# hukaixuan19970627/yolov5_obb

Measured on AMD Instinct MI355X. Metric: val.py img/s (hot path: non_max_suppression_obb, bs16) + NMS ms/img @100k cand, DOTAv1.5 1024^2, 1/2/4/8 GPU, higher is better.
Workload: dtype f16; 1 GPU; DOTAv1.5 1024^2 bs16 (BASELINE metric; configs[1] thresholds): yolov5 OBB head output (16,64512,201) fp16, 4 distinct tensors rotated (cold: 1.66 GB working set) -> non_max_suppression_obb (conf .25, iou .45, multi_label, max_det 1500), val.py --task speed hot path = dt[2] of val.py; global_batch=16, anchors_per_image=64512, nc=16, detections_per_batch=3734, parallelism=dp1 (images sharded, no data-path collective)

## Files before the change

yolov5_obb_amd/csrc/obb_device.h:

```cpp
#pragma once
#include <stdint.h>

#if defined(__HIPCC__)
#include <hip/hip_runtime.h>
#define OBB_DEV __device__ __forceinline__
#define OBB_HD __host__ __device__ __forceinline__
#else
#include <math.h>
#define OBB_DEV inline
#define OBB_HD inline
#endif

namespace obb {

constexpr int kWave = 64;

constexpr float f32_next_up(float f) {
  uint32_t u = __builtin_bit_cast(uint32_t, f);
  if (f == 0.0f) return __builtin_bit_cast(float, (uint32_t)1);
  u = (f > 0.0f) ? u + 1 : u - 1;
  return __builtin_bit_cast(float, u);
}
constexpr float f32_next_down(float f) { return -f32_next_up(-f); }
constexpr float f32_ceil(double d) {
  float f = (float)d;
  return ((double)f >= d) ? f : f32_next_up(f);
}
constexpr float f32_floor(double d) {
  float f = (float)d;
  return ((double)f <= d) ? f : f32_next_down(f);
}

static_assert((double)f32_ceil(1e-6) >= 1e-6 && (double)f32_next_down(f32_ceil(1e-6)) < 1e-6, "f32_ceil");
static_assert((double)f32_floor(1e-14) <= 1e-14 && (double)f32_next_up(f32_floor(1e-14)) > 1e-14, "f32_floor");

template <typename F> OBB_HD F min_nan(F a, F b) { return (a != a || b != b) ? a + b : (b < a ? b : a); }
template <typename F> OBB_HD bool box_too_small(F w, F h) { return min_nan(w, h) < F(0.001); }

}
```

yolov5_obb_amd/csrc/riou_device.h:

```cpp
#pragma once
#include "obb_device.h"

namespace obb {

struct RBoxFeat {
  float x, y, w, h;
  float sh, cw, ch, sw;
  float r;
  float c, s;
  float area;
};

OBB_HD RBoxFeat rbox_make_feat(float x, float y, float w, float h, float a) {
  RBoxFeat f;
  double th = (double)a;
  float c2 = (float)cos(th) * 0.5f;
  float s2 = (float)sin(th) * 0.5f;
  f.x = x; f.y = y; f.w = w; f.h = h;
  f.sh = s2 * h; f.cw = c2 * w; f.ch = c2 * h; f.sw = s2 * w;
  f.c = c2 * 2.0f; f.s = s2 * 2.0f;
  f.r = sqrtf(w * w + h * h) * 0.5005f;
  f.area = w * h;
  return f;
}
// ... 182 lines not shown
    for (int j = 0; j < 4; j++) {
      float det = e2x[j] * e1y[i] - e1x[i] * e2y[j];
      if (fabsf(det) <= kDetLe) continue;
      float dx = v2x[j] - v1x[i], dy = v2y[j] - v1y[i];
      float t1 = (e2x[j] * dy - dx * e2y[j]) / det;
      float t2 = (e1x[i] * dy - dx * e1y[i]) / det;
      if (t1 >= 0.0f && t1 <= 1.0f && t2 >= 0.0f && t2 <= 1.0f) {
        if constexpr (STORE) {
          px[n * STRIDE] = v1x[i] + e1x[i] * t1;
          py[n * STRIDE] = v1y[i] + e1y[i] * t1;
        }
        n++;
      }
    }
  }
  {
    float abab = e2x[0] * e2x[0] + e2y[0] * e2y[0];
    float adad = e2x[3] * e2x[3] + e2y[3] * e2y[3];
#pragma unroll
    for (int i = 0; i < 4; i++) {
      float apx = v1x[i] - v2x[0], apy = v1y[i] - v2y[0];
      float apab = apx * e2x[0] + apy * e2y[0];
      float apad = -(apx * e2x[3] + apy * e2y[3]);
      if (apab >= 0 && apad >= 0 && apab <= abab && apad <= adad) {
        if constexpr (STORE) { px[n * STRIDE] = v1x[i]; py[n * STRIDE] = v1y[i]; }
        n++;
      }
    }
  }
  {
    float abab = e1x[0] * e1x[0] + e1y[0] * e1y[0];
    float adad = e1x[3] * e1x[3] + e1y[3] * e1y[3];
#pragma unroll
    for (int i = 0; i < 4; i++) {
      float apx = v2x[i] - v1x[0], apy = v2y[i] - v1y[0];
      float apab = apx * e1x[0] + apy * e1y[0];
      float apad = -(apx * e1x[3] + apy * e1y[3]);
      if (apab >= 0 && apad >= 0 && apab <= abab && apad <= adad) {
        if constexpr (STORE) { px[n * STRIDE] = v2x[i]; py[n * STRIDE] = v2y[i]; }
        n++;
      }
    }
  }
  return n;
}

OBB_HD int rbox_npoints(const RBoxFeat& A, const RBoxFeat& B) {
  constexpr float kAreaLt = f32_ceil(1e-14);
  if (A.area < kAreaLt || B.area < kAreaLt) return -1;
  return rbox_points<1, false>(A, B, nullptr, nullptr);
}

template <int STRIDE>
OBB_HD float rbox_iou(const RBoxFeat& A, const RBoxFeat& B, float* px, float* py) {
  constexpr float kAreaLt = f32_ceil(1e-14);
  constexpr float kCpLtNeg = f32_ceil(-1e-6);
  constexpr float kCpLt = f32_ceil(1e-6);
  constexpr float kD2Gt = f32_floor(1e-8);

  if (A.area < kAreaLt || B.area < kAreaLt) return 0.f;
  const int n = rbox_points<STRIDE, true>(A, B, px, py);

  float inter = 0.f;
  if (n > 2) {
    int t = 0;
    float tx = px[0], ty = py[0];
    for (int i = 1; i < n; i++) {
      float x = px[i * STRIDE], y = py[i * STRIDE];
      if (y < ty || (y == ty && x < tx)) { t = i; tx = x; ty = y; }
    }
    for (int i = 0; i < n; i++) { px[i * STRIDE] -= tx; py[i * STRIDE] -= ty; }
    {
      float x0 = px[0], y0 = py[0];
      px[0] = px[t * STRIDE]; py[0] = py[t * STRIDE];
      px[t * STRIDE] = x0; py[t * STRIDE] = y0;
    }
    for (int i = 1; i < n - 1; i++) {
      float qix = px[i * STRIDE], qiy = py[i * STRIDE];
      for (int j = i + 1; j < n; j++) {
        float qjx = px[j * STRIDE], qjy = py[j * STRIDE];
        float cp = qix * qjy - qjx * qiy;
        bool sw = cp < kCpLtNeg;
        if (!sw && fabsf(cp) < kCpLt) sw = (qix * qix + qiy * qiy) > (qjx * qjx + qjy * qjy);
        if (sw) {
          px[j * STRIDE] = qix; py[j * STRIDE] = qiy;
          qix = qjx; qiy = qjy;
        }
      }
      px[i * STRIDE] = qix; py[i * STRIDE] = qiy;
    }
    int k = 1;
    for (; k < n; k++) {
      float x = px[k * STRIDE], y = py[k * STRIDE];
      if (x * x + y * y > kD2Gt) break;
    }
    if (k < n) {
      px[1 * STRIDE] = px[k * STRIDE]; py[1 * STRIDE] = py[k * STRIDE];
      int m = 2;
      for (int i = k + 1; i < n; i++) {
        float qx = px[i * STRIDE], qy = py[i * STRIDE];
        while (m > 1) {
          float bx2 = px[(m - 2) * STRIDE], by2 = py[(m - 2) * STRIDE];
          float q1x = qx - bx2, q1y = qy - by2;
          float q2x = px[(m - 1) * STRIDE] - bx2, q2y = py[(m - 1) * STRIDE] - by2;
          if (q1x * q2y >= q2x * q1y) m--; else break;
        }
        px[m * STRIDE] = qx; py[m * STRIDE] = qy; m++;
      }
      if (m > 2) {
        float q0x = px[0], q0y = py[0];
        float acc = 0.f;
        float pxx = px[1 * STRIDE] - q0x, pyy = py[1 * STRIDE] - q0y;
        for (int i = 1; i < m - 1; i++) {
          float nx = px[(i + 1) * STRIDE] - q0x, ny = py[(i + 1) * STRIDE] - q0y;
          acc += fabsf(pxx * ny - nx * pyy);
          pxx = nx; pyy = ny;
        }
        inter = acc * 0.5f;
      }
    }
  }
  return inter / (A.area + B.area - inter);
}

}
```

yolov5_obb_amd/csrc/nms.hip:

```cpp
#include <hip/hip_runtime.h>
#include <cstring>
#include <stdint.h>
#include <stdlib.h>
#include <stdio.h>
#include <string.h>
#include <hip/hip_fp16.h>
#include "launch_once.h"
#include "obb_device.h"
#include "nms_core.h"
#include "nms_mk.h"
#include "obb_hip.h"
#include "psrs_sort.h"
#include "nms_small.h"
#include "segsort.h"
#include "ws_layout.h"
#include "nms_plan.h"

namespace obb {

enum { PROF_DECODE = 0, PROF_SEGSORT, PROF_PREP, PROF_STEPS, PROF_GATHER, PROF_NMS_SORT, PROF_NMS_PREP, PROF_NMS_STEPS, PROF_N };
struct ProfState {
  int on = 0;
  static constexpr int kMax = 8192;
  hipEvent_t ev0[kMax], ev1[kMax];
// ... 939 lines not shown
  if (const int rc = head_tta_build(npass, passes_host, dtype, bs, na, no, a_total, &h, nullptr)) return rc;
  return run_nms_obb(nullptr, nullptr, dtype, bs, a_total, no, conf_thres, iou_thres, classes_host, n_classes, agnostic, multi_label, max_det,
                     max_nms, max_wh, extra8, n_extra, cap_img, expected_cand, out, out_packed ? 1 : 0, out_count, status, ws, ws_size,
                     (hipStream_t)stream, state, state_bytes, nullptr, &h);
}

int obb_profile_enable(int on) {
  g_prof.on = on == 2 ? 2 : (on != 0 ? 1 : 0);
  g_prof.used = 0;
  if (g_prof.on) {
    const int want = 2048 < ProfState::kMax ? 2048 : ProfState::kMax;
    while (g_prof.created < want) {
      if (hipEventCreate(&g_prof.ev0[g_prof.created]) != hipSuccess) return OBB_ERR_INTERNAL;
      if (hipEventCreate(&g_prof.ev1[g_prof.created]) != hipSuccess) { hipEventDestroy(g_prof.ev0[g_prof.created]); return OBB_ERR_INTERNAL; }
      g_prof.created++;
    }
  }
  return OBB_OK;
}

int obb_profile_collect(double* ms_sum, int64_t* count, int n_stages) {
  for (int i = 0; i < n_stages; i++) { ms_sum[i] = 0.0; count[i] = 0; }
  for (int k = 0; k < g_prof.used; k++) {
    float ms = 0.f;
    if (hipEventSynchronize(g_prof.ev1[k]) != hipSuccess) return OBB_ERR_INTERNAL;
    if (hipEventElapsedTime(&ms, g_prof.ev0[k], g_prof.ev1[k]) != hipSuccess) return OBB_ERR_INTERNAL;
    const int id = g_prof.id[k];
    if (id < n_stages) { ms_sum[id] += ms; count[id]++; }
  }
  g_prof.used = 0;
  return OBB_OK;
}

int obb_nms_set_max_grid(int max_workgroups) {
  g_max_grid = max_workgroups > 0 ? max_workgroups : 0;
  return OBB_OK;
}

const char* obb_version(void) { return "obb_hip 0.2 (gfx950)"; }

int obb_device_info(int* cu_count, int* wave_size, char* arch_name, int arch_name_len) {
  int dev = 0;
  if (hipGetDevice(&dev) != hipSuccess) return OBB_ERR_NO_DEVICE;
  hipDeviceProp_t p;
  if (hipGetDeviceProperties(&p, dev) != hipSuccess) return OBB_ERR_NO_DEVICE;
  if (cu_count) *cu_count = p.multiProcessorCount;
  if (wave_size) *wave_size = p.warpSize;
  if (arch_name && arch_name_len > 0) { strncpy(arch_name, p.gcnArchName, arch_name_len - 1); arch_name[arch_name_len - 1] = 0; }
  return OBB_OK;
}

}

#ifdef OBB_SMALL_TRACE
extern "C" int obb_debug_small_trace2(unsigned long long* words) {
  static unsigned long long zero2[2048 * 8];
  if (hipDeviceSynchronize() != hipSuccess) return -1;
  if (hipMemcpyFromSymbol(words, HIP_SYMBOL(obb::g_small_trace2), sizeof(obb::g_small_trace2)) != hipSuccess) return -1;
  return hipMemcpyToSymbol(HIP_SYMBOL(obb::g_small_trace2), zero2, sizeof(obb::g_small_trace2)) == hipSuccess ? 0 : -1;
}
extern "C" int obb_debug_small_trace(unsigned long long* seg_words, unsigned long long* tail_words) {
  if (hipDeviceSynchronize() != hipSuccess) return -1;
  if (hipMemcpyFromSymbol(seg_words, HIP_SYMBOL(obb::g_small_trace), sizeof(obb::g_small_trace)) != hipSuccess) return -2;
  if (hipMemcpyFromSymbol(tail_words, HIP_SYMBOL(obb::g_small_trace_tail), sizeof(obb::g_small_trace_tail)) != hipSuccess) return -3;
  static unsigned long long zero[2048 * 16];
  if (hipMemcpyToSymbol(HIP_SYMBOL(obb::g_small_trace), zero, sizeof(obb::g_small_trace)) != hipSuccess) return -4;
  if (hipMemcpyToSymbol(HIP_SYMBOL(obb::g_small_trace_tail), zero, sizeof(obb::g_small_trace_tail)) != hipSuccess) return -5;
  return 0;
}
#endif
```

yolov5_obb_amd/csrc/nms_plan.h:

```cpp
#pragma once
#include <stddef.h>
#include <stdint.h>
#include <stdlib.h>

#include "nms_limits.h"
#include "ws_layout.h"

namespace obb {

enum FbWord {
  kFbSteps = 0,
  kFbKept = 1,
  kFbSlabs = 2,
  kFbEnqueued = 3,
  kFbTicksPersist = 4,
  kFbTicksMk = 5,
  kFbKeptPersist = 6,
  kFbKeptMk = 7,
  kFbWords = 8
};
struct FbSnapshot { int w[kFbWords]; };
static inline FbSnapshot fb_snapshot(const int* words) {
  FbSnapshot s;
  for (int i = 0; i < kFbWords; i++) s.w[i] = *(const volatile int*)(words + i);
// ... 123 lines not shown
    p.slab_cap = sparse ? 2048 : 1024;
  }
  return p;
}

struct SmallHelpBlocks { int *work, *seg_np, *seg_ticket; unsigned long long *part_main, *part_help; };
static inline SmallHelpBlocks small_help_layout(WsCursor& w, int helpers, int64_t nseg, int64_t n_pos) {
  SmallHelpBlocks b;
  b.work = w.take<int>((size_t)helpers);
  b.seg_np = w.take<int>((size_t)nseg); b.seg_ticket = w.take<int>((size_t)nseg);
  b.part_main = w.take<unsigned long long>((size_t)n_pos * kSmallWords);
  b.part_help = w.take<unsigned long long>((size_t)helpers * kSmallMax * kSmallWords);
  return b;
}
static inline size_t small_help_bytes(int helpers, int64_t nseg, int64_t n_pos) {
  WsCursor w(nullptr);
  small_help_layout(w, helpers, nseg, n_pos);
  return w.total();
}

struct ObbPlanIn {
  int64_t bs, A;
  int nc, agnostic, multi_label;
  float iou_thres, max_wh;
  int64_t n_extra;
  int64_t cap_img;
  int64_t max_nms, max_det;
  int64_t expected_cand;
  int out_packed;
  int hw_cus, cus;
  long long ecap;
  size_t sort_tmp_bytes;
  size_t ps_scratch_bytes;
};
struct ObbPlan {
  int ncs;
  int class_ok;
  int multi_label;
  int64_t expected_cand, seg_hint;
  int small_hint;
  int lds_sort;
  int small_nms;
  int self_sort;
  int helpers;
  int fused_out;
  int rows_per_thread;
  int parts;
  int plan_nb, plan_chunk;
  int64_t max_seg;
  unsigned radix_mask;
  int psrs;
  unsigned gparts;
  int window;
};

static inline ObbPlan plan_nms_obb(const ObbPlanIn& in, const NmsEnv& env) {
  ObbPlan p{};
  const int64_t bs = in.bs, cap_img = in.cap_img;
  p.seg_hint = (in.expected_cand >> 32) & 0x1fffffff;
  p.small_hint = ((in.expected_cand >> 62) & 1) != 0;
  p.expected_cand = in.expected_cand & 0xffffffffll;
  p.ncs = in.agnostic ? 1 : in.nc;
  const int64_t nseg = bs * p.ncs;
  p.class_ok = (!in.agnostic && in.nc > 1 && in.A + in.n_extra < (1ll << 24) && in.iou_thres >= 0.f && in.max_wh > 0.f) ? 1 : 0;
  p.multi_label = (in.multi_label && in.nc > 1) ? 1 : 0;
  p.lds_sort = p.expected_cand > 0 && p.expected_cand <= kSortLdsHint;
  p.rows_per_thread = (bs * in.A >= 4LL * kDecThreads * 480) ? 4 : (bs * in.A >= 2LL * kDecThreads * 480) ? 2 : 1;
  p.max_seg = (in.max_nms > 0 && in.max_nms < cap_img) ? in.max_nms : cap_img;
  p.window = nms_window(in.max_det);
  const int nms_capmax = cap_max(nseg);
  p.plan_chunk = kCapFirst < nms_capmax ? kCapFirst : nms_capmax;
  p.small_nms = p.lds_sort && p.class_ok && p.seg_hint > 0 && p.seg_hint <= kSmallMax && in.iou_thres >= 0.f && nseg <= 65535;
  p.plan_nb = (nseg > 1 && !p.small_nms) ? nms_grid(nseg, bs * p.max_seg, kCapFirst, in.cus) : 0;
  const bool self_possible = p.small_nms && !in.out_packed && (int64_t)p.ncs * kSmallMax <= cap_img && env.self_sort != 0;
  if (p.small_nms && !(self_possible && env.self_sort == 2 && env.small_helpers < 0)) {
    const int64_t free_cus = (int64_t)in.hw_cus - nseg;
    p.helpers = env.small_helpers >= 0 ? env.small_helpers : (int)(free_cus < 0 ? 0 : (free_cus > kSmallHelpMax ? kSmallHelpMax : free_cus));
  }
  if (p.helpers > 0) {
    const size_t have = (size_t)(nseg < (int64_t)in.cus ? nseg : (int64_t)in.cus) * (size_t)in.ecap * 4;
    if (small_help_bytes(p.helpers, nseg, bs * cap_img) > have) p.helpers = 0;
  }
  p.self_sort = self_possible && p.helpers == 0;
  if (p.lds_sort) {
    if (!p.self_sort) p.parts = (p.class_ok && p.ncs >= 8) ? 4 : 1;
  } else {
    int tb = 0;
    while ((1ll << tb) < in.A * in.nc + in.n_extra + 1) tb++;
    unsigned mask = 0xF0u;
    for (int d = 0; d < 4; d++) if (tb > d * 8) mask |= 1u << d;
    if (p.class_ok) mask = 0xFFu;
    p.radix_mask = mask;
    p.psrs = bs == 1 && cap_img <= kPsMaxN && in.sort_tmp_bytes >= in.ps_scratch_bytes;
  }
  p.fused_out = p.small_nms && !in.out_packed;
  if (!p.fused_out)
    p.gparts = p.expected_cand <= 2048 ? 1u : (unsigned)((p.expected_cand + 1023) / 1024 > 16 ? 16 : (p.expected_cand + 1023) / 1024);
  return p;
}

}
```

yolov5_obb_amd/csrc/nmsobb_impl.h:

```cpp
#pragma once
#include "dtype_device.h"
#include "obb_device.h"
#include "segsort.h"
#include "nms_plan.h"

namespace obb {

struct ClassMask { unsigned long long w[4]; int all; };

template <typename T> __device__ __forceinline__ float mul_in_dtype(float a, float b);
template <> __device__ __forceinline__ float mul_in_dtype<float>(float a, float b) { return a * b; }
template <> __device__ __forceinline__ float mul_in_dtype<__half>(float a, float b) { return __half2float(__float2half_rn(a * b)); }
template <> __device__ __forceinline__ float mul_in_dtype<bf16_t>(float a, float b) { return round_to_dtype<bf16_t>(a * b); }
template <typename T> __device__ __forceinline__ float thr_in_dtype(float t);
template <> __device__ __forceinline__ float thr_in_dtype<float>(float t) { return t; }
template <> __device__ __forceinline__ float thr_in_dtype<__half>(float t) { return __half2float(__float2half_rn(t)); }
template <> __device__ __forceinline__ float thr_in_dtype<bf16_t>(float t) { return round_to_dtype<bf16_t>(t); }

__device__ __forceinline__ unsigned long long argmax_key(float v, int i) {
  const uint32_t b = __float_as_uint(v + 0.0f);
  const uint32_t m = (v != v) ? 0xFFFFFFFFu : (b & 0x80000000u) ? ~b : (b | 0x80000000u);
  return ((unsigned long long)m << 32) | (unsigned long long)(0xFFFFFFFFu - (uint32_t)i);
}
template <int CTRL>
// ... 26 lines not shown
}
__device__ __forceinline__ void wave_argmax_first(float& v, int& i) {
  argmax_unkey(wave_max_u64(argmax_key(v, i)), v, i);
}

struct DecodeArgs {
  const void* pred;
  const void* objcol;
  long long A;
  int no, nc, bs;
  float conf_thres;
  int multi_label;
  int rows_per_thread;
  ClassMask cm;
  long long cap_img;
  float4* cand;
  unsigned long long* keys;
  uint32_t* vals;
  int* cnt;
  int* tiny;
  float win_lo, win_hi;
  int* z_ticket; int n_ticket;
  uint4* z_bar16; long long n_bar16;
  uint4* z_alive16; long long n_alive16;
};

constexpr int kImgSmall = 1, kImgWide = 2, kImgChecked = 4, kImgCross = 8;
__host__ __device__ __forceinline__ bool img_single_list(int t) {
  return (t & kImgWide) || ((t & kImgSmall) && (!(t & kImgChecked) || (t & kImgCross)));
}
__device__ __forceinline__ int cand_flags(float x, float l, float s, float win_lo, float win_hi) {
  const float mn = min_nan(l, s);
  const float rr = sqrtf(l * l + s * s) * 0.501f + 0.5f;
  int f = (mn >= 0.001f && mn < 1.0f) ? kImgSmall : 0;
  if (!(x - rr > win_lo && x + rr < win_hi)) f |= kImgWide;
  return f;
}

__device__ __forceinline__ bool class_allowed(const ClassMask& cm, int c) {
  const int q = (c >> 6) & 3;
  const unsigned long long w = q == 0 ? cm.w[0] : q == 1 ? cm.w[1] : q == 2 ? cm.w[2] : cm.w[3];
  return cm.all || ((w >> (c & 63)) & 1ull);
}

constexpr int kCntPad = 64;

constexpr int kDecWaves = kDecThreads / 64;
constexpr int kDecMaxG = 4;
constexpr int kDecDepth = 2;
constexpr int kDecStage = 128;

constexpr int kDecCslRegs = 12;
constexpr int kDecClsRegs = 2;
template <typename T>
struct DecQuad {
  float csl[kDecCslRegs];
  float cls[kDecClsRegs];
  float box[4];
  float obj;
  uint32_t row;
  bool valid;
};

template <typename T>
__device__ __forceinline__ DecQuad<T> dec_load_quad(const T* img, int no, int nc, const uint32_t* s_row, const float* s_obj,
                                                    int j, int n_rows, int l16) {
  DecQuad<T> r;
  r.valid = j < n_rows;
  r.row = r.valid ? s_row[j] : 0u;
  r.obj = r.valid ? s_obj[j] : 0.f;
  const T* base = img + (size_t)r.row * no;
  const T* csl = base + 5 + nc;
#pragma unroll
  for (int k = 0; k < kDecCslRegs; k++) {
    const int bin = k * 16 + l16;
    r.csl[k] = (r.valid && bin < 180) ? ld_as_float<T>(csl + bin) : -__builtin_inff();
  }
#pragma unroll
  for (int g = 0; g < kDecClsRegs; g++) {
    const int c = g * 16 + l16;
    r.cls[g] = (r.valid && c < nc) ? ld_as_float<T>(base + 5 + c) : 0.f;
  }
#pragma unroll
  for (int k = 0; k < 4; k++) r.box[k] = r.valid ? ld_as_float<T>(base + k) : 0.f;
  return r;
}

template <typename T>
__global__ __launch_bounds__(kDecThreads) void k_decode(DecodeArgs a) {
  __shared__ float4 s_c0[kDecWaves][kDecStage], s_c1[kDecWaves][kDecStage];
  __shared__ unsigned long long s_key[kDecWaves][kDecStage];
  __shared__ int s_cnt[kDecWaves], s_base, s_n;
  __shared__ uint32_t s_row[kDecThreads * kDecMaxG];
  __shared__ float s_obj[kDecThreads * kDecMaxG];

  const T* pred = (const T*)a.pred;
  const int tid = threadIdx.x, lane = tid & 63, wv = tid >> 6;
  const int b = blockIdx.y;
  const int G = a.rows_per_thread;
  const float thr = thr_in_dtype<T>(a.conf_thres);
  const T* img = pred + (size_t)b * a.A * a.no;
  float4* cand = a.cand + (size_t)b * a.cap_img * 2;
  unsigned long long* keys = a.keys + (size_t)b * a.cap_img;
  uint32_t* vals = a.vals + (size_t)b * a.cap_img;
  float4* c0s = s_c0[wv]; float4* c1s = s_c1[wv]; unsigned long long* kys = s_key[wv];
  int staged = 0;
  int flags_seen = 0;
  if (tid == 0) s_n = 0;
  if (a.z_ticket != nullptr) {
    const long long i = ((long long)blockIdx.y * gridDim.x + blockIdx.x) * kDecThreads + tid, n = (long long)gridDim.x * gridDim.y * kDecThreads;
    if (i < a.n_ticket) a.z_ticket[i] = 0;
    for (long long k = i; k < a.n_bar16; k += n) a.z_bar16[k] = make_uint4(0u, 0u, 0u, 0u);
    for (long long k = i; k < a.n_alive16; k += n) a.z_alive16[k] = make_uint4(0u, 0u, 0u, 0u);
  }
  __syncthreads();

  auto write_out = [&](long long base, int count) {
    for (int i = lane; i < count; i += 64) {
      const long long slot = base + i;
      if (slot < a.cap_img) {
        cand[slot * 2] = c0s[i];
        cand[slot * 2 + 1] = c1s[i];
        keys[slot] = kys[i];
        vals[slot] = (uint32_t)slot;
      }
    }
  };
  auto flush_wave = [&]() {
    int base = 0;
    if (lane == 0) base = atomicAdd(&a.cnt[b * kCntPad], staged);
    base = __shfl(base, 0);
    write_out(base, staged);
    staged = 0;
  };

  float obj[kDecMaxG];
  auto row_of = [&](int q) -> long long { return ((long long)(q * (kDecThreads / 16) + (tid >> 4)) * gridDim.x + blockIdx.x) * 16 + (tid & 15); };
#pragma unroll
  for (int q = 0; q < kDecMaxG; q++) {
    const long long row = row_of(q);
    obj[q] = (q >= G || row >= a.A) ? 0.f
             : a.objcol ? ld_as_float<T>((const T*)a.objcol + (size_t)b * a.A + row)
                        : ld_as_float<T>(img + (size_t)row * a.no + 4);
  }
#pragma unroll
  for (int q = 0; q < kDecMaxG; q++) {
    const bool p = q < G && row_of(q) < a.A && obj[q] > thr;
    const unsigned long long mk = __ballot(p);
    if (mk) {
      int base = 0;
      if (lane == 0) base = atomicAdd(&s_n, __popcll(mk));
      base = __shfl(base, 0);
      if (p) {
        const int i = base + __popcll(mk & lanemask_lt());
        s_row[i] = (uint32_t)row_of(q);
        s_obj[i] = obj[q];
      }
    }
  }
  __syncthreads();
  const int n_rows = s_n;

  const int l16 = lane & 15, sub = lane >> 4;
  const int ncg = (a.nc + 15) >> 4;
  auto reduce_quad = [&](const DecQuad<T>& cur) {
    unsigned long long tk = argmax_key(cur.csl[0], l16);
#pragma unroll
    for (int k = 1; k < kDecCslRegs; k++) { const unsigned long long kk = argmax_key(cur.csl[k], k * 16 + l16); tk = kk > tk ? kk : tk; }
    float tv; int ti;
    argmax_unkey(row_max_u64(tk), tv, ti);
    const float theta = ((float)(ti - 90) / 180.0f) * 3.141592f;
    const float bx = cur.box[0], by = cur.box[1], bl = cur.box[2], bs_ = cur.box[3];
    const int bflags = cand_flags(bx, bl, bs_, a.win_lo, a.win_hi);
    const long long rw = (long long)cur.row;
    auto stage = [&](bool p, float conf, int c) {
      const unsigned long long pb = __ballot(p);
      const int np = __popcll(pb);
      if (np == 0) return;
      if (staged + np > kDecStage) flush_wave();
      if (p) {
        const int i = staged + __popcll(pb & lanemask_lt());
        c0s[i] = make_float4(bx, by, bl, bs_);
        c1s[i] = make_float4(theta, conf, (float)c, 0.f);
        kys[i] = ((unsigned long long)score_desc_key(conf) << 32) | (unsigned long long)(uint32_t)(rw * a.nc + c);
        flags_seen |= bflags;
      }
      staged += np;
    };
    unsigned long long bestk = argmax_key(-__builtin_inff(), 0x7fffffff);
    for (int g = 0; g < ncg; g++) {
      const int c = g * 16 + l16;
      float raw;
      if (g < kDecClsRegs) raw = (g == 0) ? cur.cls[0] : cur.cls[1];
      else raw = (cur.valid && c < a.nc) ? ld_as_float<T>(img + (size_t)cur.row * a.no + 5 + c) : 0.f;
      const float v = (cur.valid && c < a.nc) ? mul_in_dtype<T>(raw, cur.obj) : -__builtin_inff();
      if (a.multi_label) stage(cur.valid && c < a.nc && v > thr && class_allowed(a.cm, c), v, c);
      else if (c < a.nc) { const unsigned long long kk = argmax_key(v, c); bestk = kk > bestk ? kk : bestk; }
    }
    if (!a.multi_label) {
      float bv; int bi;
      argmax_unkey(row_max_u64(bestk), bv, bi);
      stage(cur.valid && l16 == 0 && bv > thr && class_allowed(a.cm, bi), bv, bi);
    }
  };
  static_assert(kDecClsRegs == 2, "reduce_quad selects cls[0] / cls[1] explicitly");
  for (int g0 = wv; g0 * 4 < n_rows; g0 += kDecWaves * kDecDepth) {
    DecQuad<T> quads[kDecDepth];
#pragma unroll
    for (int i = 0; i < kDecDepth; i++) {
      const int g = g0 + kDecWaves * i;
      if (g * 4 < n_rows) quads[i] = dec_load_quad<T>(img, a.no, a.nc, s_row, s_obj, g * 4 + sub, n_rows, l16);
    }
#pragma unroll
    for (int i = 0; i < kDecDepth; i++) {
      const int g = g0 + kDecWaves * i;
      if (g * 4 < n_rows) reduce_quad(quads[i]);
    }
  }

  {
    const int fl = (__ballot(flags_seen & kImgSmall) ? kImgSmall : 0) | (__ballot(flags_seen & kImgWide) ? kImgWide : 0);
    if (fl && lane == 0) atomicOr(&a.tiny[b], fl);
  }
  if (lane == 0) s_cnt[wv] = staged;
  __syncthreads();
  if (threadIdx.x == 0) {
    int tot = 0;
    for (int w = 0; w < kDecWaves; w++) tot += s_cnt[w];
    s_base = tot ? atomicAdd(&a.cnt[b * kCntPad], tot) : 0;
  }
  __syncthreads();
  int base = s_base;
  for (int w = 0; w < wv; w++) base += s_cnt[w];
  write_out(base, staged);
}

__global__ void k_append_extra(const float* __restrict__ extra8, int m, long long A, int nc, DecodeArgs a) {
  int i = blockIdx.x * blockDim.x + threadIdx.x;
  if (i >= m) return;
  const float* e = extra8 + (size_t)i * 8;
  const int b = (int)e[0];
  if (b < 0 || b >= a.bs) return;
  if (!(e[6] > a.conf_thres) || !class_allowed(a.cm, (int)e[7])) return;
  const int slot = atomicAdd(&a.cnt[b * kCntPad], 1);
  { const int fl = cand_flags(e[1], e[3], e[4], a.win_lo, a.win_hi); if (fl) atomicOr(&a.tiny[b], fl); }
  if (slot >= a.cap_img) return;
  const size_t g = (size_t)b * a.cap_img + slot;
  a.cand[g * 2] = make_float4(e[1], e[2], e[3], e[4]);
  a.cand[g * 2 + 1] = make_float4(e[5], e[6], e[7], 0.f);
  a.keys[g] = ((unsigned long long)score_desc_key(e[6]) << 32) | (unsigned long long)(uint32_t)(A * nc + i);
  a.vals[g] = (uint32_t)slot;
}

constexpr int kTinyMax = 64;
constexpr long long kTinyPairs = 262144;
constexpr int kTinyParts = 32;
__global__ __launch_bounds__(256) void k_tiny_cross(const float4* __restrict__ cand, const unsigned long long* __restrict__ keys,
                                                    const int* __restrict__ cnt, long long cap_img, float class_offset, float thr,
                                                    int* __restrict__ tiny) {
  __shared__ float scr[RotGeom::SCR * 256];
  __shared__ RBoxFeat s_feat[kTinyMax];
  __shared__ unsigned long long s_key[kTinyMax];
  __shared__ float s_cls[kTinyMax];
  __shared__ int s_list[kTinyMax];
  __shared__ int s_n;
  const int b = blockIdx.y, part = blockIdx.x, tid = threadIdx.x, lane = tid & 63, wv = tid >> 6;
  if ((tiny[b] & (kImgSmall | kImgWide)) != kImgSmall) return;
  long long n = cnt[b * kCntPad];
  if (n > cap_img) n = cap_img;
  const size_t base = (size_t)b * cap_img;
  if (tid == 0) s_n = 0;
  __syncthreads();
  for (long long j = tid; j < n; j += 256) {
    const float4 c0 = cand[(base + j) * 2];
    const float mn = min_nan(c0.z, c0.w);
    if (mn >= 0.001f && mn < 1.0f) { const int k = atomicAdd(&s_n, 1); if (k < kTinyMax) s_list[k] = (int)j; }
  }
  __syncthreads();
  const int nt = s_n;
  if (nt > kTinyMax || (long long)nt * n > kTinyPairs) return;
  if (part == 0 && tid == 0) atomicOr(&tiny[b], kImgChecked);
  for (int t = tid; t < nt; t += 256) {
    const int jt = s_list[t];
    const float4 t0 = cand[(base + jt) * 2], t1 = cand[(base + jt) * 2 + 1];
    const float offT = t1.z * class_offset;
    s_feat[t] = rbox_make_feat(t0.x + offT, t0.y + offT, t0.z, t0.w, t1.x);
    s_key[t] = keys[base + jt];
// ... 837 lines not shown
  w.nest([&](void* b) { return (cv.nms = carve(b, (int64_t)n, bs * ncs, RotGeom::RECQ, cap_max(bs * ncs))).total; });
  cv.total = w.total();
  return cv;
}

struct HeadFront;
struct HeadFrontTta;
static int launch_decode_head(const HeadFront& h, const DecodeArgs& d, int dtype, hipStream_t st);
static int launch_decode_head_tta(const HeadFrontTta& h, const DecodeArgs& d, int dtype, hipStream_t st);

static int run_nms_obb(const void* pred, const void* objcol, int dtype, int64_t bs, int64_t A, int64_t no, float conf_thres, float iou_thres,
                       const int32_t* classes_host, int n_classes, int agnostic, int multi_label, int64_t max_det, int64_t max_nms,
                       float max_wh, const float* extra8, int64_t n_extra, int64_t cap_img, int64_t expected_cand, float* out,
                       int out_packed, int64_t* out_count, int64_t* status, void* ws, size_t ws_bytes, hipStream_t st, void* state = nullptr,
                       size_t state_bytes = 0, const HeadFront* head = nullptr, const HeadFrontTta* tta = nullptr) {
  const int nc = (int)(no - 5 - 180);
  if (bs < 1 || A < 1 || nc < 1 || nc > 256 || max_det < 1 || cap_img < 1 || (!pred && !head && !tta) || !out || !out_count || !status)
    return OBB_ERR_BAD_ARG;
  if (A * nc + n_extra > 0xffffffffLL || bs * cap_img > 0x7fffffffLL) return OBB_ERR_BAD_ARG;
  if (!dtype_known(dtype)) return OBB_ERR_BAD_ARG;
  cap_img = round_cap(cap_img);
  ObbCarve cv = obb_carve(ws, bs, cap_img, agnostic ? 1 : nc);
  if (!ws_ok(ws, ws_bytes, cv.total)) return OBB_ERR_WORKSPACE;
  ObbPlanIn pin{};
  pin.bs = bs; pin.A = A; pin.nc = nc; pin.agnostic = agnostic; pin.multi_label = multi_label; pin.iou_thres = iou_thres; pin.max_wh = max_wh;
  pin.n_extra = n_extra; pin.cap_img = cap_img; pin.max_nms = max_nms; pin.max_det = max_det; pin.expected_cand = expected_cand;
  pin.out_packed = out_packed; pin.hw_cus = hw_cu_count(); pin.cus = cu_count(); pin.ecap = cv.nms.ecap;
  pin.sort_tmp_bytes = cv.nms.sort_tmp_bytes; pin.ps_scratch_bytes = ps_scratch_bytes();
  const ObbPlan plan = plan_nms_obb(pin, nms_env());
  const int ncs = plan.ncs, class_ok = plan.class_ok, helpers = plan.helpers;
  int rc = OBB_OK;
  const bool kept = state != nullptr;
  if (kept) {
    if (!ws_ok(state, state_bytes, obb_state_bytes(bs))) return OBB_ERR_WORKSPACE;
    cv.cnt = (int*)state;
    cv.tiny = cv.cnt + bs * kCntPad;
  }

  DecodeArgs d;
  d.pred = pred; d.objcol = objcol; d.A = A; d.no = (int)no; d.nc = nc; d.bs = (int)bs; d.conf_thres = conf_thres;
  d.multi_label = plan.multi_label;
  d.cm.all = (classes_host == nullptr || n_classes <= 0) ? 1 : 0;
  for (int i = 0; i < 4; i++) d.cm.w[i] = 0ull;
  for (int i = 0; i < n_classes && classes_host; i++) {
    int c = classes_host[i];
    if (c >= 0 && c < 256) d.cm.w[c >> 6] |= 1ull << (c & 63);
  }
  d.cap_img = cap_img; d.cand = cv.cand; d.keys = cv.keys_a; d.vals = cv.vals_a; d.cnt = cv.cnt; d.tiny = cv.tiny;
  d.win_lo = -0.35f * max_wh; d.win_hi = 0.6f * max_wh;

  d.z_ticket = nullptr; d.n_ticket = 0; d.z_bar16 = nullptr; d.n_bar16 = 0; d.z_alive16 = nullptr; d.n_alive16 = 0;
  {
    Carve& nv0 = cv.nms;
    const long long alive16 = plan.lds_sort ? (long long)((((size_t)bs * cap_img) >> 6) + 8 + 1) / 2 : 0ll;
    if (kept) {
      d.z_ticket = cv.ticket; d.n_ticket = (int)(16 + bs + 1);
      d.z_bar16 = reinterpret_cast<uint4*>(nv0.bar); d.n_bar16 = (long long)(nv0.bar_bytes / 16);
      d.z_alive16 = reinterpret_cast<uint4*>(nv0.alive); d.n_alive16 = alive16;
    } else {
      k_reset_state<<<256, 256, 0, st>>>(cv.cnt, (int)(bs * kCntPad), cv.tiny, (int)bs, status, cv.ticket, (int)(16 + bs + 1),
                                         reinterpret_cast<uint4*>(nv0.bar), (long long)(nv0.bar_bytes / 16),
                                         reinterpret_cast<uint4*>(nv0.alive), alive16);
    }
  }
  d.rows_per_thread = plan.rows_per_thread;
  dim3 gd((unsigned)((A + kDecThreads * d.rows_per_thread - 1) / (kDecThreads * d.rows_per_thread)), (unsigned)bs);
  {
    ProfScope ps(PROF_DECODE, st);
    if (head || tta) {
      rc = head ? launch_decode_head(*head, d, dtype, st) : launch_decode_head_tta(*tta, d, dtype, st);
      if (rc) return rc;
    } else OBB_DISPATCH_DTYPE(dtype, T, k_decode<T><<<gd, kDecThreads, 0, st>>>(d));
  }
  if (n_extra > 0 && extra8) k_append_extra<<<(unsigned)((n_extra + 255) / 256), 256, 0, st>>>(extra8, (int)n_extra, A, nc, d);
  if (plan.small_hint && class_ok)
    k_tiny_cross<<<dim3(kTinyParts, (unsigned)bs), 256, 0, st>>>(cv.cand, cv.keys_a, cv.cnt, cap_img, max_wh, iou_thres, cv.tiny);
  const unsigned gs = (unsigned)((bs + 255) / 256);
  Carve& nv = cv.nms;
  const int64_t max_seg = plan.max_seg;
  SmallHelpBlocks hb{};
  if (helpers > 0) { WsCursor w(nv.edges); hb = small_help_layout(w, helpers, bs * ncs, bs * cap_img); }
  if (plan.self_sort) {
  } else if (plan.lds_sort) {
    ProfScope ps(PROF_SEGSORT, st);
    static OncePerDevice attr;
    const size_t lds = (size_t)kSortLdsMax * 12;
    if (const int attr_dev = attr.need(); attr_dev != OncePerDevice::kDone) {
      if (hipFuncSetAttribute((const void*)k_sort_prep_lds, hipFuncAttributeMaxDynamicSharedMemorySize, (int)lds) != hipSuccess)
        return OBB_ERR_LAUNCH;
      attr.mark(attr_dev);
    }
    k_sort_prep_lds<<<(unsigned)(bs * plan.parts) + (plan.plan_nb > 0 ? 1u : 0u), 1024, lds, st>>>(cv.cand, cv.keys_a, cv.vals_a, cv.keys_b, cv.vals_b, cv.cnt, cv.tiny, (int)bs, cap_img,
                                                   max_nms, class_ok, A, nc, ncs, agnostic ? 0.f : max_wh, cv.sort_begin, cv.sort_end,
                                                   cv.img_end, cv.mode, nv.seg_begin, nv.seg_end, nv.keep_cnt,
                                                   nv.rec, nv.alive, cv.ticket, plan.plan_nb, plan.plan_chunk, plan.plan_nb > 0 ? nv.plan : nullptr,
                                                   cv.seg_size, plan.parts,
                                                   helpers, hb.work, hb.seg_np, hb.seg_ticket);
  } else {
   {
    ProfScope ps(PROF_SEGSORT, st);
    k_cand_segments<<<gs, 256, 0, st>>>(cv.cnt, cv.tiny, (int)bs, cap_img, max_nms, class_ok, cv.sort_begin, cv.sort_end, cv.img_end,
                                        cv.mode);
    if (class_ok) {
      dim3 gr((unsigned)((cap_img + 255) / 256), (unsigned)bs);
      k_rekey<<<gr, 256, 0, st>>>(cv.cand, cv.keys_a, cv.sort_begin, cv.sort_end, cv.mode, A, nc);
    }
    {
      if (plan.psrs) {
        PsBuf b{};
        b.run_k = cv.keys_a; b.run_v = cv.vals_a; b.out_k = cv.keys_b; b.out_v = cv.vals_b;
        b.n = (int)cap_img; b.n_dev = cv.sort_end; b.err = nullptr;
        ps_carve_scratch(nv.sort_tmp, &b);
        const int runs = (int)((cap_img + kPsRun - 1) / kPsRun);
        k_ps_local_pairs<<<(unsigned)runs, kPsRun, 0, st>>>(b, cv.keys_a, cv.vals_a);
        rc = ps_finish(b, runs, st);
// ... 73 lines not shown
```

Baseline: 142,500 img/s.

## Compute rotated-box intersection area in registers with branchless sorting networks

Adds a register-resident version of the polygon-area step in rotated IoU. It loads the intersection points into fixed-size arrays, finds the pivot, sorts by angle with a predicated compare-swap network and builds the convex hull with select operations. A wave-wide ballot chooses an 8-point or 6-point variant so every lane in the wave runs the same path, and the scalar loop is kept for more than 8 points. The goal is to avoid scratch-memory accesses and divergent data-dependent loops, at the cost of more registers, extra fixed work per lane and a noinline call.

```diff
diff --git a/yolov5_obb_amd/csrc/obb_device.h b/yolov5_obb_amd/csrc/obb_device.h
--- a/yolov5_obb_amd/csrc/obb_device.h
+++ b/yolov5_obb_amd/csrc/obb_device.h
@@ -5,10 +5,12 @@
 #include <hip/hip_runtime.h>
 #define OBB_DEV __device__ __forceinline__
 #define OBB_HD __host__ __device__ __forceinline__
+#define OBB_HD_FN __host__ __device__ __attribute__((noinline))
 #else
 #include <math.h>
 #define OBB_DEV inline
 #define OBB_HD inline
+#define OBB_HD_FN inline
 #endif
 
 namespace obb {
diff --git a/yolov5_obb_amd/csrc/riou_device.h b/yolov5_obb_amd/csrc/riou_device.h
--- a/yolov5_obb_amd/csrc/riou_device.h
+++ b/yolov5_obb_amd/csrc/riou_device.h
@@ -258,14 +258,10 @@
 }
 
 template <int STRIDE>
-OBB_HD float rbox_iou(const RBoxFeat& A, const RBoxFeat& B, float* px, float* py) {
-  constexpr float kAreaLt = f32_ceil(1e-14);
+OBB_HD float rbox_inter_loop(int n, float* px, float* py) {
   constexpr float kCpLtNeg = f32_ceil(-1e-6);
   constexpr float kCpLt = f32_ceil(1e-6);
   constexpr float kD2Gt = f32_floor(1e-8);
-
-  if (A.area < kAreaLt || B.area < kAreaLt) return 0.f;
-  const int n = rbox_points<STRIDE, true>(A, B, px, py);
 
   float inter = 0.f;
   if (n > 2) {
@@ -326,7 +322,131 @@
       }
     }
   }
-  return inter / (A.area + B.area - inter);
-}
-
-}
+  return inter;
+}
+
+template <int NR, int STRIDE>
+OBB_HD_FN float rbox_inter_reg(int n, const float* px, const float* py) {
+  static_assert(NR >= 3 && NR <= 24, "rbox_inter_reg: NR");
+  constexpr float kCpLtNeg = f32_ceil(-1e-6);
+  constexpr float kCpLt = f32_ceil(1e-6);
+  constexpr float kD2Gt = f32_floor(1e-8);
+
+  float x[NR], y[NR], d[NR];
+#pragma unroll
+  for (int i = 0; i < NR; i++) { x[i] = px[i * STRIDE]; y[i] = py[i * STRIDE]; }
+  if (n <= 2) return 0.f;
+#pragma unroll
+  for (int i = 3; i < NR; i++) {
+    x[i] = i < n ? x[i] : 0.f; y[i] = i < n ? y[i] : 0.f;
+  }
+
+  int t = 0;
+  float tx = x[0], ty = y[0];
+#pragma unroll
+  for (int i = 1; i < NR; i++) {
+    const bool lower = (i < n) & ((y[i] < ty) | ((y[i] == ty) & (x[i] < tx)));
+    t = lower ? i : t; tx = lower ? x[i] : tx; ty = lower ? y[i] : ty;
+  }
+#pragma unroll
+  for (int i = 0; i < NR; i++) { x[i] -= tx; y[i] -= ty; }
+  {
+    const float x0 = x[0], y0 = y[0];
+#pragma unroll
+    for (int i = 1; i < NR; i++) {
+      const bool piv = t == i;
+      x[0] = piv ? x[i] : x[0]; y[0] = piv ? y[i] : y[0];
+      x[i] = piv ? x0 : x[i];   y[i] = piv ? y0 : y[i];
+    }
+  }
+#pragma unroll
+  for (int i = 0; i < NR; i++) d[i] = x[i] * x[i] + y[i] * y[i];
+
+#pragma unroll
+  for (int i = 1; i < NR - 1; i++) {
+#pragma unroll
+    for (int j = i + 1; j < NR; j++) {
+      const float cp = x[i] * y[j] - x[j] * y[i];
+      const bool sw = (j < n) & ((cp < kCpLtNeg) | ((fabsf(cp) < kCpLt) & (d[i] > d[j])));
+      const float xi = x[i], yi = y[i], di = d[i], xj = x[j], yj = y[j], dj = d[j];
+      x[i] = sw ? xj : xi; y[i] = sw ? yj : yi; d[i] = sw ? dj : di;
+      x[j] = sw ? xi : xj; y[j] = sw ? yi : yj; d[j] = sw ? di : dj;
+    }
+  }
+
+  int k = n;
+#pragma unroll
+  for (int i = NR - 1; i >= 1; i--) k = ((i < n) & (d[i] > kD2Gt)) ? i : k;
+  if (k >= n) return 0.f;
+
+  float hx[NR], hy[NR];
+#pragma unroll
+  for (int i = 0; i < NR; i++) { hx[i] = 0.f; hy[i] = 0.f; }
+  hx[0] = x[0]; hy[0] = y[0];
+#pragma unroll
+  for (int i = 1; i < NR; i++) { hx[1] = k == i ? x[i] : hx[1]; hy[1] = k == i ? y[i] : hy[1]; }
+  float ax = hx[0], ay = hy[0], bx = hx[1], by = hy[1];
+  int m = 2;
+#pragma unroll
+  for (int i = 2; i < NR; i++) {
+    const bool act = (i > k) & (i < n);
+    const float qx = x[i], qy = y[i];
+    for (;;) {
+      const float q1x = qx - ax, q1y = qy - ay;
+      const float q2x = bx - ax, q2y = by - ay;
+      if (!(act & (m > 1) & (q1x * q2y >= q2x * q1y))) break;
+      m--;
+      bx = ax; by = ay;
+#pragma unroll
+      for (int j = 0; j <= i - 3; j++) {
+        ax = m - 2 == j ? hx[j] : ax; ay = m - 2 == j ? hy[j] : ay;
+      }
+    }
+#pragma unroll
+    for (int j = 1; j <= i; j++) {
+      const bool put = act & (m == j);
+      hx[j] = put ? qx : hx[j]; hy[j] = put ? qy : hy[j];
+    }
+    ax = act ? bx : ax; ay = act ? by : ay; bx = act ? qx : bx; by = act ? qy : by;
+    m += act ? 1 : 0;
+  }
+  if (m <= 2) return 0.f;
+
+  const float q0x = hx[0], q0y = hy[0];
+  float acc = 0.f;
+  float pxx = hx[1] - q0x, pyy = hy[1] - q0y;
+#pragma unroll
+  for (int i = 1; i < NR - 1; i++) {
+    const float nx = hx[i + 1] - q0x, ny = hy[i + 1] - q0y;
+    const float term = fabsf(pxx * ny - nx * pyy);
+    acc = i < m - 1 ? acc + term : acc;
+    pxx = nx; pyy = ny;
+  }
+  return acc * 0.5f;
+}
+
+template <int STRIDE>
+OBB_HD float rbox_iou(const RBoxFeat& A, const RBoxFeat& B, float* px, float* py) {
+  constexpr float kAreaLt = f32_ceil(1e-14);
+
+  if (A.area < kAreaLt || B.area < kAreaLt) return 0.f;
+  const int n = rbox_points<STRIDE, true>(A, B, px, py);
+  const float area12 = A.area + B.area;
+
+  float inter = 0.f;
+  if (n > 2) {
+    if (n <= 8) {
+#if defined(__HIP_DEVICE_COMPILE__)
+      const bool wide = __builtin_amdgcn_ballot_w64(n > 6) != 0;
+#else
+      const bool wide = n > 6;
+#endif
+      inter = wide ? rbox_inter_reg<8, STRIDE>(n, px, py) : rbox_inter_reg<6, STRIDE>(n, px, py);
+    } else {
+      inter = rbox_inter_loop<STRIDE>(n, px, py);
+    }
+  }
+  return inter / (area12 - inter);
+}
+
+}
```

Measured after the change: 143,200 img/s, median of 6. No clear change (+0.5%).

## Trim decode kernel zeroing and predicated loads, hoist objectness loads before scratch clearing

Applied to the files above, without the earlier changes.

Zeroing of the NMS barrier and alive scratch now happens only when the plan says later stages need it, via new zero_bar/zero_alive flags. In the decode kernel the objectness loads are issued before the scratch-clearing stores so their latency overlaps the clears. Per-row loads are made unconditional with clamped or fallback addresses so the compiler can drop predication, and the staging lambdas are restructured. It also adds optional wall-clock tracing macros behind a compile flag. The risk is that skipping the clears leaves stale scratch if the plan predicates are wrong for some configuration.

```diff
diff --git a/yolov5_obb_amd/csrc/nms.hip b/yolov5_obb_amd/csrc/nms.hip
--- a/yolov5_obb_amd/csrc/nms.hip
+++ b/yolov5_obb_amd/csrc/nms.hip
@@ -1015,6 +1015,15 @@
 
 }
 
+#ifdef OBB_DECODE_TRACE
+extern "C" int obb_debug_decode_trace(unsigned long long* words) {
+  static unsigned long long zero[obb::kDecTraceWgs * 16];
+  if (hipDeviceSynchronize() != hipSuccess) return -1;
+  if (hipMemcpyFromSymbol(words, HIP_SYMBOL(obb::g_decode_trace), sizeof(obb::g_decode_trace)) != hipSuccess) return -2;
+  return hipMemcpyToSymbol(HIP_SYMBOL(obb::g_decode_trace), zero, sizeof(obb::g_decode_trace)) == hipSuccess ? 0 : -3;
+}
+#endif
+
 #ifdef OBB_SMALL_TRACE
 extern "C" int obb_debug_small_trace2(unsigned long long* words) {
   static unsigned long long zero2[2048 * 8];
diff --git a/yolov5_obb_amd/csrc/nms_plan.h b/yolov5_obb_amd/csrc/nms_plan.h
--- a/yolov5_obb_amd/csrc/nms_plan.h
+++ b/yolov5_obb_amd/csrc/nms_plan.h
@@ -199,6 +199,8 @@
   int psrs;
   unsigned gparts;
   int window;
+  int zero_bar;
+  int zero_alive;
 };
 
 static inline ObbPlan plan_nms_obb(const ObbPlanIn& in, const NmsEnv& env) {
@@ -243,6 +245,8 @@
   p.fused_out = p.small_nms && !in.out_packed;
   if (!p.fused_out)
     p.gparts = p.expected_cand <= 2048 ? 1u : (unsigned)((p.expected_cand + 1023) / 1024 > 16 ? 16 : (p.expected_cand + 1023) / 1024);
+  p.zero_bar = (!p.small_nms || !p.fused_out) ? 1 : 0;
+  p.zero_alive = (p.lds_sort && !p.self_sort) ? 1 : 0;
   return p;
 }
 
diff --git a/yolov5_obb_amd/csrc/nmsobb_impl.h b/yolov5_obb_amd/csrc/nmsobb_impl.h
--- a/yolov5_obb_amd/csrc/nmsobb_impl.h
+++ b/yolov5_obb_amd/csrc/nmsobb_impl.h
@@ -102,6 +102,26 @@
 
 constexpr int kDecCslRegs = 12;
 constexpr int kDecClsRegs = 2;
+#ifdef OBB_DECODE_TRACE
+constexpr int kDecTraceWgs = 2048;
+__device__ unsigned long long g_decode_trace[kDecTraceWgs * 16];
+#define DTRACE_DECL() __shared__ unsigned long long s_tr[16]; if (threadIdx.x < 16) s_tr[threadIdx.x] = (threadIdx.x == 3 || threadIdx.x == 6) ? ~0ull : 0ull; \
+  if (threadIdx.x == 0) s_tr[1] = wall_clock64()
+#define DTRACE_T0(slot) do { if (threadIdx.x == 0) s_tr[slot] = wall_clock64(); } while (0)
+#define DTRACE_WAVE(slot_min, slot_max) do { if ((threadIdx.x & 63) == 0) { const unsigned long long t_ = wall_clock64(); \
+  atomicMin(&s_tr[slot_min], t_); atomicMax(&s_tr[slot_max], t_); } } while (0)
+#define DTRACE_ADD(slot, v) do { if ((threadIdx.x & 63) == 0) atomicAdd(&s_tr[slot], (unsigned long long)(v)); } while (0)
+#define DTRACE_END(n_rows) do { DTRACE_WAVE(15, 9); __syncthreads(); \
+  const unsigned wg_ = blockIdx.y * gridDim.x + blockIdx.x; \
+  if (threadIdx.x < 16 && wg_ < (unsigned)kDecTraceWgs) g_decode_trace[wg_ * 16 + threadIdx.x] = threadIdx.x == 0 ? 1ull : threadIdx.x == 10 ? (unsigned long long)(n_rows) : s_tr[threadIdx.x]; } while (0)
+#else
+#define DTRACE_DECL() do {} while (0)
+#define DTRACE_T0(slot) do {} while (0)
+#define DTRACE_WAVE(slot_min, slot_max) do {} while (0)
+#define DTRACE_ADD(slot, v) do {} while (0)
+#define DTRACE_END(n_rows) do {} while (0)
+#endif
+
 template <typename T>
 struct DecQuad {
   float csl[kDecCslRegs];
@@ -119,20 +139,14 @@
   r.valid = j < n_rows;
   r.row = r.valid ? s_row[j] : 0u;
   r.obj = r.valid ? s_obj[j] : 0.f;
-  const T* base = img + (size_t)r.row * no;
+  const T* base = img + (size_t)r.row * (uint32_t)no;
   const T* csl = base + 5 + nc;
 #pragma unroll
-  for (int k = 0; k < kDecCslRegs; k++) {
-    const int bin = k * 16 + l16;
-    r.csl[k] = (r.valid && bin < 180) ? ld_as_float<T>(csl + bin) : -__builtin_inff();
-  }
-#pragma unroll
-  for (int g = 0; g < kDecClsRegs; g++) {
-    const int c = g * 16 + l16;
-    r.cls[g] = (r.valid && c < nc) ? ld_as_float<T>(base + 5 + c) : 0.f;
-  }
-#pragma unroll
-  for (int k = 0; k < 4; k++) r.box[k] = r.valid ? ld_as_float<T>(base + k) : 0.f;
+  for (int k = 0; k < kDecCslRegs; k++) r.csl[k] = ld_as_float<T>((k * 16 + l16 < 180) ? csl + k * 16 + l16 : base);
+#pragma unroll
+  for (int g = 0; g < kDecClsRegs; g++) r.cls[g] = ld_as_float<T>((g * 16 + l16 < nc) ? base + 5 + g * 16 + l16 : base);
+#pragma unroll
+  for (int k = 0; k < 4; k++) r.box[k] = ld_as_float<T>(base + k);
   return r;
 }
 
@@ -157,13 +171,7 @@
   int staged = 0;
   int flags_seen = 0;
   if (tid == 0) s_n = 0;
-  if (a.z_ticket != nullptr) {
-    const long long i = ((long long)blockIdx.y * gridDim.x + blockIdx.x) * kDecThreads + tid, n = (long long)gridDim.x * gridDim.y * kDecThreads;
-    if (i < a.n_ticket) a.z_ticket[i] = 0;
-    for (long long k = i; k < a.n_bar16; k += n) a.z_bar16[k] = make_uint4(0u, 0u, 0u, 0u);
-    for (long long k = i; k < a.n_alive16; k += n) a.z_alive16[k] = make_uint4(0u, 0u, 0u, 0u);
-  }
-  __syncthreads();
+  DTRACE_DECL();
 
   auto write_out = [&](long long base, int count) {
     for (int i = lane; i < count; i += 64) {
@@ -186,13 +194,21 @@
 
   float obj[kDecMaxG];
   auto row_of = [&](int q) -> long long { return ((long long)(q * (kDecThreads / 16) + (tid >> 4)) * gridDim.x + blockIdx.x) * 16 + (tid & 15); };
+  const T* ocol = a.objcol ? (const T*)a.objcol + (size_t)b * a.A : img + 4;
+  const long long ostride = a.objcol ? 1 : a.no;
 #pragma unroll
   for (int q = 0; q < kDecMaxG; q++) {
     const long long row = row_of(q);
-    obj[q] = (q >= G || row >= a.A) ? 0.f
-             : a.objcol ? ld_as_float<T>((const T*)a.objcol + (size_t)b * a.A + row)
-                        : ld_as_float<T>(img + (size_t)row * a.no + 4);
-  }
+    obj[q] = ld_as_float<T>(ocol + (size_t)(row < a.A ? row : a.A - 1) * ostride);
+  }
+  if (a.z_ticket != nullptr) {
+    const long long i = ((long long)blockIdx.y * gridDim.x + blockIdx.x) * kDecThreads + tid, n = (long long)gridDim.x * gridDim.y * kDecThreads;
+    if (i < a.n_ticket) a.z_ticket[i] = 0;
+    for (long long k = i; k < a.n_bar16; k += n) a.z_bar16[k] = make_uint4(0u, 0u, 0u, 0u);
+    for (long long k = i; k < a.n_alive16; k += n) a.z_alive16[k] = make_uint4(0u, 0u, 0u, 0u);
+  }
+  __syncthreads();
+  DTRACE_T0(2);
 #pragma unroll
   for (int q = 0; q < kDecMaxG; q++) {
     const bool p = q < G && row_of(q) < a.A && obj[q] > thr;
@@ -208,35 +224,52 @@
       }
     }
   }
+  DTRACE_WAVE(3, 4);
   __syncthreads();
+  DTRACE_T0(5);
   const int n_rows = s_n;
 
   const int l16 = lane & 15, sub = lane >> 4;
   const int ncg = (a.nc + 15) >> 4;
-  auto reduce_quad = [&](const DecQuad<T>& cur) {
-    unsigned long long tk = argmax_key(cur.csl[0], l16);
-#pragma unroll
-    for (int k = 1; k < kDecCslRegs; k++) { const unsigned long long kk = argmax_key(cur.csl[k], k * 16 + l16); tk = kk > tk ? kk : tk; }
+  struct RowOut { float bx, by, bl, bs_, theta; int bflags; long long rw; };
+  auto stage = [&](const RowOut& o, bool p, float conf, int c) {
+    const unsigned long long pb = __ballot(p);
+    const int np = __popcll(pb);
+    if (np == 0) return;
+    if (staged + np > kDecStage) flush_wave();
+    if (p) {
+      const int i = staged + __popcll(pb & lanemask_lt());
+      c0s[i] = make_float4(o.bx, o.by, o.bl, o.bs_);
+      c1s[i] = make_float4(o.theta, conf, (float)c, 0.f);
+      kys[i] = ((unsigned long long)score_desc_key(conf) << 32) | (unsigned long long)(uint32_t)(o.rw * a.nc + c);
+      flags_seen |= o.bflags;
+    }
+    staged += np;
+    DTRACE_ADD(11, np);
+  };
+  auto row_out = [&](float bx, float by, float bl, float bs_, unsigned long long tk, uint32_t row) {
     float tv; int ti;
     argmax_unkey(row_max_u64(tk), tv, ti);
-    const float theta = ((float)(ti - 90) / 180.0f) * 3.141592f;
-    const float bx = cur.box[0], by = cur.box[1], bl = cur.box[2], bs_ = cur.box[3];
-    const int bflags = cand_flags(bx, bl, bs_, a.win_lo, a.win_hi);
-    const long long rw = (long long)cur.row;
-    auto stage = [&](bool p, float conf, int c) {
-      const unsigned long long pb = __ballot(p);
-      const int np = __popcll(pb);
-      if (np == 0) return;
-      if (staged + np > kDecStage) flush_wave();
-      if (p) {
-        const int i = staged + __popcll(pb & lanemask_lt());
-        c0s[i] = make_float4(bx, by, bl, bs_);
-        c1s[i] = make_float4(theta, conf, (float)c, 0.f);
-        kys[i] = ((unsigned long long)score_desc_key(conf) << 32) | (unsigned long long)(uint32_t)(rw * a.nc + c);
-        flags_seen |= bflags;
-      }
-      staged += np;
-    };
+    RowOut o;
+    o.bx = bx; o.by = by; o.bl = bl; o.bs_ = bs_;
+    o.theta = ((float)(ti - 90) / 180.0f) * 3.141592f;
+    o.bflags = cand_flags(bx, bl, bs_, a.win_lo, a.win_hi);
+    o.rw = (long long)row;
+    return o;
+  };
+  auto stage_best = [&](const RowOut& o, bool valid, unsigned long long bestk) {
+    float bv; int bi;
+    argmax_unkey(row_max_u64(bestk), bv, bi);
+    stage(o, valid && l16 == 0 && bv > thr && class_allowed(a.cm, bi), bv, bi);
+  };
+  auto reduce_quad = [&](const DecQuad<T>& cur) __attribute__((always_inline)) {
+    unsigned long long tk = argmax_key(cur.csl[0], l16);
+#pragma unroll
+    for (int k = 1; k < kDecCslRegs; k++) {
+      const unsigned long long kk = (k * 16 + l16 < 180) ? argmax_key(cur.csl[k], k * 16 + l16) : 0ull;
+      tk = kk > tk ? kk : tk;
+    }
+    const RowOut o = row_out(cur.box[0], cur.box[1], cur.box[2], cur.box[3], tk, cur.row);
     unsigned long long bestk = argmax_key(-__builtin_inff(), 0x7fffffff);
     for (int g = 0; g < ncg; g++) {
       const int c = g * 16 + l16;
@@ -244,14 +277,10 @@
       if (g < kDecClsRegs) raw = (g == 0) ? cur.cls[0] : cur.cls[1];
       else raw = (cur.valid && c < a.nc) ? ld_as_float<T>(img + (size_t)cur.row * a.no + 5 + c) : 0.f;
       const float v = (cur.valid && c < a.nc) ? mul_in_dtype<T>(raw, cur.obj) : -__builtin_inff();
-      if (a.multi_label) stage(cur.valid && c < a.nc && v > thr && class_allowed(a.cm, c), v, c);
+      if (a.multi_label) stage(o, cur.valid && c < a.nc && v > thr && class_allowed(a.cm, c), v, c);
       else if (c < a.nc) { const unsigned long long kk = argmax_key(v, c); bestk = kk > bestk ? kk : bestk; }
     }
-    if (!a.multi_label) {
-      float bv; int bi;
-      argmax_unkey(row_max_u64(bestk), bv, bi);
-      stage(cur.valid && l16 == 0 && bv > thr && class_allowed(a.cm, bi), bv, bi);
-    }
+    if (!a.multi_label) stage_best(o, cur.valid, bestk);
   };
   static_assert(kDecClsRegs == 2, "reduce_quad selects cls[0] / cls[1] explicitly");
   for (int g0 = wv; g0 * 4 < n_rows; g0 += kDecWaves * kDecDepth) {
@@ -272,6 +301,7 @@
     const int fl = (__ballot(flags_seen & kImgSmall) ? kImgSmall : 0) | (__ballot(flags_seen & kImgWide) ? kImgWide : 0);
     if (fl && lane == 0) atomicOr(&a.tiny[b], fl);
   }
+  DTRACE_WAVE(6, 7);
   if (lane == 0) s_cnt[wv] = staged;
   __syncthreads();
   if (threadIdx.x == 0) {
@@ -280,9 +310,11 @@
     s_base = tot ? atomicAdd(&a.cnt[b * kCntPad], tot) : 0;
   }
   __syncthreads();
+  DTRACE_T0(8);
   int base = s_base;
   for (int w = 0; w < wv; w++) base += s_cnt[w];
   write_out(base, staged);
+  DTRACE_END(n_rows);
 }
 
 __global__ void k_append_extra(const float* __restrict__ extra8, int m, long long A, int nc, DecodeArgs a) {
@@ -1226,15 +1258,15 @@
   d.z_ticket = nullptr; d.n_ticket = 0; d.z_bar16 = nullptr; d.n_bar16 = 0; d.z_alive16 = nullptr; d.n_alive16 = 0;
   {
     Carve& nv0 = cv.nms;
-    const long long alive16 = plan.lds_sort ? (long long)((((size_t)bs * cap_img) >> 6) + 8 + 1) / 2 : 0ll;
+    const long long alive16 = plan.zero_alive ? (long long)((((size_t)bs * cap_img) >> 6) + 8 + 1) / 2 : 0ll;
+    const long long bar16 = plan.zero_bar ? (long long)(nv0.bar_bytes / 16) : 0ll;
     if (kept) {
       d.z_ticket = cv.ticket; d.n_ticket = (int)(16 + bs + 1);
-      d.z_bar16 = reinterpret_cast<uint4*>(nv0.bar); d.n_bar16 = (long long)(nv0.bar_bytes / 16);
-      d.z_alive16 = reinterpret_cast<uint4*>(nv0.alive); d.n_alive16 = alive16;
+      d.z_bar16 = bar16 ? reinterpret_cast<uint4*>(nv0.bar) : nullptr; d.n_bar16 = bar16;
+      d.z_alive16 = alive16 ? reinterpret_cast<uint4*>(nv0.alive) : nullptr; d.n_alive16 = alive16;
     } else {
       k_reset_state<<<256, 256, 0, st>>>(cv.cnt, (int)(bs * kCntPad), cv.tiny, (int)bs, status, cv.ticket, (int)(16 + bs + 1),
-                                         reinterpret_cast<uint4*>(nv0.bar), (long long)(nv0.bar_bytes / 16),
-                                         reinterpret_cast<uint4*>(nv0.alive), alive16);
+                                         reinterpret_cast<uint4*>(nv0.bar), bar16, reinterpret_cast<uint4*>(nv0.alive), alive16);
     }
   }
   d.rows_per_thread = plan.rows_per_thread;
```

Measured after the change: 142,700 img/s before, 157,700 img/s after, median of 6. 10.5% higher.
